# SAIC-MONTREAL/multimodal-dynamics

Measured on AMD Instinct MI355X. Metric: visuotactile samples/sec (train) + ELBO vs CPU ref, cnn-mvae 64x64 bs256 @1/2/4/8 GPU, higher is better.
Workload: dtype f32x3; 1 GPU; cnn-mvae visuotactile+pose 64x64, bs=256 per GPU, fp32 storage and results, GEMMs in the fp32x3 arithmetic (exact three-term bf16 split of the fp32 operands, six of nine products on the bf16 matrix cores, fp32 accumulate; error vs fp64 <= native fp32 MFMA), seq_modeling train step (7 subset ELBOs + backward + Adam), BASELINE configs[1]; global_batch=256, parallelism=dp1, bn=local, launch=hip_graph

## Files before the change

### include/mmdyn_hip.h

```cpp
#ifndef MMDYN_HIP_H
#define MMDYN_HIP_H

#include <stdint.h>

#ifdef __cplusplus
extern "C" {
#endif

#define MMDYN_OK 0
#define MMDYN_ERR_SHAPE (-1)
#define MMDYN_ERR_NULL (-2)
#define MMDYN_ERR_RANGE (-3)

#define MMDYN_ACT_NONE 0
#define MMDYN_ACT_SWISH 1
#define MMDYN_ACT_RELU 2

#define MMDYN_DENSE 0
#define MMDYN_CONV 1
#define MMDYN_TCONV_S2P1 2
#define MMDYN_IM2COL3 3

#define MMDYN_TCONV_S1P0 4

// ... 12 lines not shown
int mmdyn_igemm_nt_dgrad_bn(const float* A, const float* Bp, float* C, float* stats, const float* y,
                            const float* mean, const float* rstd, const float* gamma, const float* beta,
                            int mode, int G, int Bg, int Hi, int Wi, int Cin, int Ho, int Wo, int N,
                            int stride, int offset, int bf16, float* ws, uint32_t* arrival_flags, void* stream);
int mmdyn_igemm_slab_floats(int mode, int G, int Bg, int Hi, int Wi, int Cin, int Ho, int Wo, int N);

int mmdyn_igemm_nt_bf16(const float* A, const float* Bp, const float* bias, float* C, float* C_act,
                        float* stats, float* ws, int mode, int G, int Bg, int Hi, int Wi, int Cin,
                        int Ho, int Wo, int N, int ldc, int stride, int offset, int act, int splitk,
                        void* stream);
int mmdyn_igemm_nt_f16(const float* A, const float* Bp, const float* bias, float* C, float* C_act,
                       float* stats, float* ws, int mode, int G, int Bg, int Hi, int Wi, int Cin,
                       int Ho, int Wo, int N, int ldc, int stride, int offset, int act, int splitk,
                       void* stream);
int mmdyn_igemm_stat_tiles(int mode, int G, int Bg, int Hi, int Wi, int Cin, int Ho, int Wo, int N);
int mmdyn_igemm_stat_tiles_bf16(int mode, int G, int Bg, int Hi, int Wi, int Cin, int Ho, int Wo, int N);
int mmdyn_igemm_stat_tiles_mx(int mode, int G, int Bg, int Hi, int Wi, int Cin, int Ho, int Wo, int N, int flags);
int mmdyn_igemm_slab_floats_mx(int mode, int G, int Bg, int Hi, int Wi, int Cin, int Ho, int Wo, int N, int flags);
int mmdyn_igemm_nt_grouped(const void* A, const void* Bp, const float* bias, void* C, void* C_act, const void* u, int G,
                           int rows, int K, int N, int act, int flags, void* stream);
int mmdyn_splitk_reduce(const float* ws, const float* bias, float* C, float* C_act, int splitk,
                        int rows, int N, int act, void* stream);

int mmdyn_wgrad_tn(const float* D, const float* Gt, float* partial, int mode, int Bt, int Hr, int Wr,
                   int Cd, int Hi, int Wi, int Cg, int stride, int offset, int chunks, void* stream);
int mmdyn_wgrad_tn_bf16(const float* D, const float* Gt, float* partial, int mode, int Bt, int Hr, int Wr,
                        int Cd, int Hi, int Wi, int Cg, int stride, int offset, int chunks, void* stream);
int mmdyn_wgrad_tn_f16(const float* D, const float* Gt, float* partial, int mode, int Bt, int Hr, int Wr,
                       int Cd, int Hi, int Wi, int Cg, int stride, int offset, int chunks, void* stream);
int mmdyn_wgrad_tn_grouped(const void* D, const void* Gt, float* partial, int G, int rows, int Cd, int Cg, int chunks,
                           int flags, void* stream);
int mmdyn_wgrad_out3_bn(const void* y, const float* mean, const float* rstd, const float* gamma, const float* beta,
                        const float* Gt, float* partial, int G, int Bg, int Hr, int chunks, int y_b16, void* stream);
int mmdyn_wgrad_chunks(int mode, int rows, int Cd, int Cg);
int mmdyn_wgrad_chunks_mx(int mode, int rows, int Cd, int Cg, int flags);
int mmdyn_wgrad_reduce(const float* partial, float* canon, int chunks, int taps, int Cd, int Cg,
                       int cg_canon, int perm, float beta, void* stream);

int mmdyn_pack_conv_weight(const float* Wc, float* P, int d0, int d1, int swap, void* stream);
int mmdyn_repack2d(const float* in, float* out, int rows_in, int cols_in, int rows_out, int cols_out,
                   int mode, void* stream);

int mmdyn_repack2d_ld(const float* in, float* out, int rows_in, int cols_in, int rows_out, int cols_out,
                      int ld_out, int mode, void* stream);
int mmdyn_pack_conv_weight_b16(const float* Wc, void* P, int d0, int d1, int swap, int half, void* stream);
int mmdyn_repack2d_ld_b16(const float* in, void* out, int rows_in, int cols_in, int rows_out, int cols_out,
                          int ld_out, int mode, int half, void* stream);
typedef struct {
  const float* src;
  float* dst;
  int kind, rows_in, cols_in, rows_out, cols_out, ld_out;
  int dst_bf16;
} mmdyn_pack_entry;
int mmdyn_pack_plan(const mmdyn_pack_entry* plan_dev, int n, void* stream);

int mmdyn_im2col_nchw3(const float* x, float* col, int Bt, int H, int W, void* stream);
int mmdyn_col2im_k4(const float* col, float* out, int Bt, int Hi, int Wi, int Ho, int Wo, int C,
                    int ldcol, int stride, int pad, int tap_major, void* stream);

int mmdyn_tconv_out3_fwd(const float* a, const float* w, float* out, int Bt, int Hi, int Wi, void* stream);
int mmdyn_tconv_out3_bn_fwd(const void* y, const float* mean, const float* rstd, const float* gamma, const float* beta,
                            const float* w, float* out, int G, int Bg, int Hi, int Wi, int b16, void* stream);
int mmdyn_tconv_out3_bn_bce(const void* y, const float* mean, const float* rstd, const float* gamma, const float* beta,
                            const float* w, float* logits, int logits_group, const float* target, const float* mask,
                            int mask_channels, float* dlogit, double* loss_slots, double* unmasked_slots,
                            const int* slot_of_group, float grad_scale, int G, int Bg, int Hi, int Wi, int b16, void* stream);
// ... 204 lines not shown
```

### multimodal-dynamics_amd/csrc/conv3.hip

```cpp
#include "common.h"

namespace {

struct Conv3Geom {
  int G, Bg, Hi, Wi, Ho, ldc;
  int act, want_act_out, want_stats, w_b16;
  int tiles_per_group;
  const void* bn_y;
  const float* bn_mean;
  const float* bn_rstd;
  const float* bn_gamma;
  const float* bn_beta;
};

#define GLOBAL_AS __attribute__((address_space(1)))
typedef GLOBAL_AS char* gchar_p;
__device__ __forceinline__ gchar_p sgpr_ptr(const void* p) {
  const uint64_t u = reinterpret_cast<uint64_t>(p);
  const uint32_t lo = __builtin_amdgcn_readfirstlane((uint32_t)u), hi = __builtin_amdgcn_readfirstlane((uint32_t)(u >> 32));
  return (gchar_p)(((uint64_t)hi << 32) | lo);
}
template <typename T> __device__ __forceinline__ float gld1(gchar_p p);
template <> __device__ __forceinline__ float gld1<float>(gchar_p p) { return *(GLOBAL_AS const float*)p; }
template <> __device__ __forceinline__ float gld1<bf16_t>(gchar_p p) {
  return __uint_as_float((uint32_t)(*(GLOBAL_AS const bf16_t*)p) << 16);
}
template <> __device__ __forceinline__ float gld1<half_t>(gchar_p p) { return h2f(*(GLOBAL_AS const uint16_t*)p); }
template <typename T> struct store16 { typedef bf16_t type; };
template <> struct store16<half_t> { typedef half_t type; };

constexpr int C3_N = 32;
template <typename T, bool BN, int ACT, int SEGS>
__global__ __launch_bounds__(256) __attribute__((amdgpu_waves_per_eu(4, 4))) void conv3_nt_kernel(
    const float* __restrict__ img, const float* __restrict__ Wp, T* __restrict__ C, T* __restrict__ C_act,
    float* __restrict__ stats, const Conv3Geom g) {
  __shared__ float Ws[32 * 65];
  __shared__ float red[4][2][32];
  const int tid = threadIdx.x, lane = tid & 63;
  const int wave = __builtin_amdgcn_readfirstlane(tid >> 6);
  const int x = lane & 31, h = lane >> 5;
  for (int i = tid; i < 512; i += 256) {
    const f32x4 v = g.w_b16 == 2 ? ld4<half_t>(reinterpret_cast<const half_t*>(Wp) + 4 * i)
                    : g.w_b16 ? ld4<bf16_t>(reinterpret_cast<const bf16_t*>(Wp) + 4 * i)
                              : reinterpret_cast<const f32x4*>(Wp)[i];
    const int n = i >> 4, k = (i & 15) * 4;
    Ws[n * 65 + k + 0] = v[0];
    Ws[n * 65 + k + 1] = v[1];
    Ws[n * 65 + k + 2] = v[2];
    Ws[n * 65 + k + 3] = v[3];
  }
  __syncthreads();
  float bw[24];
  auto load_bw = [&]() {
#pragma unroll
    for (int j = 0; j < 24; ++j) bw[j] = Ws[x * 65 + (j >> 3) * 16 + ((j >> 1) & 3) * 4 + 2 * (j & 1) + h];
  };
  if (!BN) load_bw();

  const float bn_g = BN ? g.bn_gamma[x] : 0.f, bn_b = BN ? g.bn_beta[x] : 0.f;
  const int ntiles = g.G * g.tiles_per_group;

  constexpr int C3_HI = 64 * SEGS, C3_HO = 32 * SEGS;
  constexpr int UNITS = C3_HO * SEGS;
  int xl[2];
#pragma unroll
  for (int q = 0; q < 2; ++q) xl[q] = 2 * x - 1 + 2 * q + h;
  const unsigned voffB = (4 * h * C3_N + x) * sizeof(T);
  constexpr unsigned IMG_B = 3 * C3_HI * C3_HI * sizeof(float);
  constexpr unsigned OROW_B = 32 * C3_N * sizeof(T);

  struct TileAt {
    gchar_p imgb;
    size_t orow;
    int y, seg;
    unsigned xoB[2];
    bool xok[2];
  };
  auto locate = [&](int t) {
    TileAt p;
    const int u = t * 4 + wave;
    const int ib = u / UNITS, rem = u - ib * UNITS;
    p.y = rem / SEGS;
    p.seg = rem - p.y * SEGS;
    p.imgb = sgpr_ptr(reinterpret_cast<const char*>(img) + (size_t)ib * IMG_B + (size_t)p.seg * 256 - 4);
    p.orow = (size_t)u * OROW_B;
#pragma unroll
    for (int q = 0; q < 2; ++q) {
      p.xok[q] = (unsigned)(p.seg * 64 + xl[q]) < (unsigned)C3_HI;
      p.xoB[q] = (unsigned)((p.xok[q] ? xl[q] + 1 : 1) * 4);
    }
    return p;
  };
  auto load_a = [&](const TileAt& p, int j) {
    const int ci = j >> 3, yin = 2 * p.y - 1 + ((j >> 1) & 3);
    const bool yok = (unsigned)yin < (unsigned)C3_HI;
    const gchar_p rowp = p.imgb + (unsigned)((ci * C3_HI + (yok ? yin : 0)) * C3_HI) * 4u;
    return gld1<float>(rowp + p.xoB[j & 1]);
  };
  auto erow = [](int e) { return (unsigned)(((e & 3) + 8 * (e >> 2)) * C3_N * sizeof(T)); };

  float a[24], yv[16];
  int t = blockIdx.x;
  if (t >= ntiles) return;
  TileAt cur = locate(t);
#pragma unroll
  for (int j = 0; j < 24; ++j) a[j] = load_a(cur, j);
  if (BN) {
    const gchar_p yb = sgpr_ptr(reinterpret_cast<const char*>(g.bn_y) + cur.orow) + voffB;
#pragma unroll
    for (int e = 0; e < 16; ++e) yv[e] = gld1<T>(yb + erow(e));
  }
  for (; t < ntiles; t += gridDim.x) {
    const int tn = t + gridDim.x < ntiles ? t + gridDim.x : t;
    const TileAt nxt = locate(tn);
    const int grp = (BN || g.want_stats) ? __builtin_amdgcn_readfirstlane((t / (UNITS / 4)) / g.Bg) : 0;
    if (BN) load_bw();
    float bn_m = 0.f, bn_r = 0.f;
    if (BN) {
      bn_m = g.bn_mean[grp * 32 + x];
      bn_r = g.bn_rstd[grp * 32 + x];
    }
    f32x16 acc;
#pragma unroll
    for (int e = 0; e < 16; ++e) acc[e] = 0.f;
#pragma unroll
    for (int j = 0; j < 24; ++j) {
      const int yin = 2 * cur.y - 1 + ((j >> 1) & 3);
      const bool ok = ((unsigned)yin < (unsigned)C3_HI) & cur.xok[j & 1];
      acc = __builtin_amdgcn_mfma_f32_32x32x2f32(ok ? a[j] : 0.f, bw[j], acc, 0, 0, 0);
      a[j] = load_a(nxt, j);
    }

    const gchar_p cb = sgpr_ptr(reinterpret_cast<const char*>(C) + cur.orow) + voffB;
    const gchar_p ab = sgpr_ptr(reinterpret_cast<const char*>(C_act) + cur.orow) + voffB;
    const gchar_p yb = sgpr_ptr(reinterpret_cast<const char*>(g.bn_y) + nxt.orow) + voffB;
    float cs = 0.f, cq = 0.f;
#pragma unroll
    for (int e = 0; e < 16; ++e) {
      float v = acc[e];
      if (BN) {
        const float xh = (yv[e] - bn_m) * bn_r;
        yv[e] = gld1<T>(yb + erow(e));
        v *= swish_gradf_(bn_g * xh + bn_b);
        cs += v;
        cq += v * xh;
      } else {
        cs += v;
        cq += v * v;
      }
      if (sizeof(T) == 2) {
        const float vn = __shfl_down(v, 1, 64);
        if (!(x & 1)) {
          *(GLOBAL_AS uint32_t*)(cb + erow(e)) = pack2<typename store16<T>::type>(v, vn);
          if (ACT >= 0)
            *(GLOBAL_AS uint32_t*)(ab + erow(e)) = pack2<typename store16<T>::type>(apply_act(v, ACT), apply_act(vn, ACT));
        }
      } else {
        *(GLOBAL_AS float*)(cb + erow(e)) = v;
        if (ACT >= 0) *(GLOBAL_AS float*)(ab + erow(e)) = apply_act(v, ACT);
      }
    }
    if (g.want_stats) {
      cs += __shfl_xor(cs, 32, 64);
      cq += __shfl_xor(cq, 32, 64);
      if (h == 0) {
        red[wave][0][x] = cs;
        red[wave][1][x] = cq;
      }
      __syncthreads();
      if (tid < 32) {
        float s0 = 0.f, q0 = 0.f;
#pragma unroll
        for (int w = 0; w < 4; ++w) {
          s0 += red[w][0][tid];
          q0 += red[w][1][tid];
        }
        const size_t sb = ((size_t)t * 2) * 32 + tid;
        stats[sb] = s0;
        stats[sb + 32] = q0;
      }
      __syncthreads();
    }
    cur = nxt;
  }
}

struct Conv3WgradGeom {
  int Bt, Hr, Hi, Wi;
  int img_rows;
  int rows_per_chunk;
  const float* bn_mean;
  const float* bn_rstd;
  const float* bn_gamma;
  const float* bn_beta;
  int Bg;
// ... 160 lines not shown
  g.bn_gamma = bn_gamma;
  g.bn_beta = bn_beta;
  const int ntiles = G * g.tiles_per_group;
  const dim3 grid(ntiles < CONV3_GRID ? ntiles : CONV3_GRID);
  const int variant = bn_y ? 4 : (C_act ? act : -1);
#define CONV3_LAUNCH(T_, BN_, ACT_, S_)                                                                            \
  hipLaunchKernelGGL((conv3_nt_kernel<T_, BN_, ACT_, S_>), grid, dim3(256), 0, st, A, Bp, (T_*)C, (T_*)C_act, stats, g)
#define CONV3_CASE(V, BN_, ACT_)                                                                                   \
  if (variant == (V)) {                                                                                            \
    if (c_b16 == 2) {                                                                                              \
      if (segs == 1) CONV3_LAUNCH(half_t, BN_, ACT_, 1);                                                           \
      else if (segs == 2) CONV3_LAUNCH(half_t, BN_, ACT_, 2);                                                      \
      else CONV3_LAUNCH(half_t, BN_, ACT_, 4);                                                                     \
    } else if (c_b16) {                                                                                            \
      if (segs == 1) CONV3_LAUNCH(bf16_t, BN_, ACT_, 1);                                                           \
      else if (segs == 2) CONV3_LAUNCH(bf16_t, BN_, ACT_, 2);                                                      \
      else CONV3_LAUNCH(bf16_t, BN_, ACT_, 4);                                                                     \
    } else {                                                                                                       \
      if (segs == 1) CONV3_LAUNCH(float, BN_, ACT_, 1);                                                            \
      else if (segs == 2) CONV3_LAUNCH(float, BN_, ACT_, 2);                                                       \
      else CONV3_LAUNCH(float, BN_, ACT_, 4);                                                                      \
    }                                                                                                              \
  }
  CONV3_CASE(4, true, -1)
  CONV3_CASE(-1, false, -1)
  CONV3_CASE(MMDYN_ACT_NONE, false, MMDYN_ACT_NONE)
  CONV3_CASE(MMDYN_ACT_SWISH, false, MMDYN_ACT_SWISH)
  CONV3_CASE(MMDYN_ACT_RELU, false, MMDYN_ACT_RELU)
#undef CONV3_LAUNCH
#undef CONV3_CASE
  MMDYN_LAUNCH_CHECK();
}

int mmdyn_conv3_wgrad_try(const void* D, const float* Gt, float* partial, int Bt, int Hr, int Wr, int Cd, int Hi,
                          int Wi, int Cg, int chunks, int d_b16, hipStream_t st, const float* bn_mean, const float* bn_rstd,
                          const float* bn_gamma, const float* bn_beta, int Bg) {
  if (Cd != 32 || Cg != 64 || Wr != Hr || Wi != Hi || Hi != 2 * Hr || (Hi != 64 && Hi != 128 && Hi != 256)) return 1;
  const int segs = Hi / 64;
  if ((int64_t)Bt * Hr * segs >= (1LL << 30)) return 1;
  Conv3WgradGeom g{};
  g.Bt = Bt;
  g.Hr = Hr;
  g.Hi = Hi;
  g.Wi = Wi;
  g.img_rows = Bt * Hr * segs;
  g.rows_per_chunk = ceil_div(g.img_rows, chunks);
  g.bn_mean = bn_mean;
  g.bn_rstd = bn_rstd;
  g.bn_gamma = bn_gamma;
  g.bn_beta = bn_beta;
  g.Bg = Bg > 0 ? Bg : Bt;
#define CONV3_WG(T_, S_)                                                                                                  \
  do {                                                                                                                    \
    if (bn_mean)                                                                                                          \
      hipLaunchKernelGGL((conv3_wgrad_kernel<T_, S_, true>), dim3(chunks), dim3(256), 0, st, (const T_*)D, Gt, partial, g); \
    else                                                                                                                  \
      hipLaunchKernelGGL((conv3_wgrad_kernel<T_, S_>), dim3(chunks), dim3(256), 0, st, (const T_*)D, Gt, partial, g);     \
  } while (0)
  if (d_b16 == 2) {
    if (segs == 1) CONV3_WG(half_t, 1);
    else if (segs == 2) CONV3_WG(half_t, 2);
    else CONV3_WG(half_t, 4);
  } else if (d_b16) {
    if (segs == 1) CONV3_WG(bf16_t, 1);
    else if (segs == 2) CONV3_WG(bf16_t, 2);
    else CONV3_WG(bf16_t, 4);
// ... 9 lines not shown
```

### multimodal-dynamics_amd/mmdyn_hip/_lib.py

```python
import ctypes
import os

_HERE = os.path.dirname(os.path.abspath(__file__))
LIB_PATH = os.environ.get("MMDYN_HIP_LIB") or os.path.join(_HERE, "libmmdyn_hip.so")

_P, _I, _L, _F, _Q = ctypes.c_void_p, ctypes.c_int, ctypes.c_int64, ctypes.c_float, ctypes.c_uint64


class PassExperts(ctypes.Structure):
    _fields_ = [("mu", _P * 4), ("lv", _P * 4), ("dmu", _P * 4), ("dlv", _P * 4), ("ld", _I * 4), ("dz", _P * 3),
                ("zdst", _P * 3), ("zpl", _P * 3)]


class PackEntry(ctypes.Structure):
    _fields_ = [("src", _P), ("dst", _P), ("kind", _I), ("rows_in", _I), ("cols_in", _I), ("rows_out", _I),
                ("cols_out", _I), ("ld_out", _I), ("dst_bf16", _I)]


class FeedGroups(ctypes.Structure):
    _fields_ = [("recon", _P * 4), ("obs", _P * 4), ("out", _P * 4), ("row_len", _I * 4), ("logits", _I * 4), ("column", _I * 4)]


MAX_PASSES = 8
MAX_EXPERTS = 4
# ... 3 lines not shown
_SIGNATURES = {
    "mmdyn_abi_version": "",
    "mmdyn_igemm_nt": "ppppppp" + "iiiiiiiiiiiiii" + "p",
    "mmdyn_igemm_nt_dgrad_bn": "ppppppppp" + "iiiiiiiiiiii" + "ppp",
    "mmdyn_igemm_nt_dgrad_act": "pppp" + "i" + "iiiiiiiiiii" + "i" + "ppp",
    "mmdyn_igemm_slab_floats": "iiiiiiiii",
    "mmdyn_igemm_nt_bf16": "ppppppp" + "iiiiiiiiiiiiii" + "p",
    "mmdyn_igemm_nt_f16": "ppppppp" + "iiiiiiiiiiiiii" + "p",
    "mmdyn_igemm_stat_tiles": "iiiiiiiii",
    "mmdyn_igemm_stat_tiles_bf16": "iiiiiiiii",
    "mmdyn_igemm_stat_tiles_mx": "iiiiiiiiii",
    "mmdyn_igemm_slab_floats_mx": "iiiiiiiiii",
    "mmdyn_igemm_nt_grouped": "pppppp" + "iiiiii" + "p",
    "mmdyn_splitk_reduce": "pppp" + "iiii" + "p",
    "mmdyn_wgrad_tn": "ppp" + "iiiiiiiiiii" + "p",
    "mmdyn_wgrad_tn_bf16": "ppp" + "iiiiiiiiiii" + "p",
    "mmdyn_wgrad_tn_f16": "ppp" + "iiiiiiiiiii" + "p",
    "mmdyn_wgrad_tn_grouped": "ppp" + "iiiiii" + "p",
    "mmdyn_wgrad_chunks": "iiii",
    "mmdyn_wgrad_chunks_mx": "iiiii",
    "mmdyn_wgrad_reduce": "pp" + "iiiiii" + "f" + "p",
    "mmdyn_pack_conv_weight": "pp" + "iii" + "p",
    "mmdyn_repack2d": "pp" + "iiiii" + "p",
    "mmdyn_repack2d_ld": "pp" + "iiiiii" + "p",
    "mmdyn_pack_conv_weight_b16": "pp" + "iiii" + "p",
    "mmdyn_repack2d_ld_b16": "pp" + "iiiiiii" + "p",
    "mmdyn_pack_plan": "p" + "i" + "p",
    "mmdyn_im2col_nchw3": "pp" + "iii" + "p",
    "mmdyn_col2im_k4": "pp" + "iiiiiiiiii" + "p",
    "mmdyn_tconv_out3_fwd": "ppp" + "iii" + "p",
    "mmdyn_tconv_out3_bn_fwd": "ppppppp" + "iiiii" + "p",
    "mmdyn_tconv_out3_bn_bce": "ppppppp" + "i" + "pp" + "i" + "pppp" + "f" + "iiiii" + "p",
    "mmdyn_wgrad_out3_bn": "ppppppp" + "iiiii" + "p",
    "mmdyn_colstats": "pp" + "iii" + "p",
    "mmdyn_colstats_tiles": "i",
    "mmdyn_bn_finalize": "ppppppp" + "iiii" + "ff" + "i" + "pp",
    "mmdyn_bn_swish_fwd": "pppppp" + "iii" + "p",
    "mmdyn_bn_swish_bwd_reduce": "ppppppp" + "iii" + "p",
    "mmdyn_bn_bwd_finalize": "ppppp" + "iii" + "f" + "pp",
    "mmdyn_bn_eval_stats": "pppp" + "ii" + "f" + "p",
    "mmdyn_bn_reduce_partials": "ppp" + "iii" + "p",
    "mmdyn_bn_finalize_sums": "pppppp" + "iii" + "ff" + "i" + "p",
    "mmdyn_bn_bwd_finalize_sums": "pppp" + "ii" + "ff" + "p",
    "mmdyn_bn_swish_bwd_apply": "pppppppp" + "iiii" + "p",
    "mmdyn_act_fwd": "pp" + "l" + "i" + "p",
    "mmdyn_act_bwd": "ppp" + "l" + "i" + "p",
    "mmdyn_dropout_expand": "ppp" + "iii" + "f" + "p",
    "mmdyn_dropout_reduce": "ppp" + "iii" + "f" + "pi" + "pp",
    "mmdyn_random_masks": "p" + "l" + "f" + "QQ" + "pp",
    "mmdyn_random_normal": "p" + "l" + "QQ" + "pp",
    "mmdyn_counter_add": "p" + "Q" + "p",
    "mmdyn_colsum": "ppp" + "iii" + "f" + "pp",
    "mmdyn_colsum_chunks": "i",
    "mmdyn_scale_dev": "ppp" + "l" + "p",
    "mmdyn_sum_blocks": "pp" + "i" + "l" + "p",
    "mmdyn_copy_many": "ppp" + "i" + "p",
    "mmdyn_cast_f32_to_bf16": "pp" + "l" + "p",
    "mmdyn_cast_bf16_to_f32": "pp" + "l" + "p",
    "mmdyn_linear_small_fwd": "pppp" + "iiii" + "p",
    "mmdyn_linear_small_bwd": "pppppp" + "iii" + "f" + "p",
    "mmdyn_poe_fwd": "pppppp" + "iiii" + "p",
    "mmdyn_poe_bwd": "ppppppp" + "f" + "iiii" + "pp",
    "mmdyn_reparam_fwd": "ppppp" + "iii" + "p",
    "mmdyn_reparam_bwd": "pppp" + "f" + "pp" + "iii" + "p",
    "mmdyn_bce_logits": "ppppp" + "l" + "iii" + "f" + "p",
    "mmdyn_bce_logits_groups": "ppppp" + "i" + "l" + "f" + "p",
# ... 89 lines not shown
```

### multimodal-dynamics_amd/mmdyn_hip/layers.py

```python
import weakref

import torch

from . import ops
from .ops import ACT_NONE, ACT_SWISH, ACT_RELU, DENSE, CONV, TCONV_S2P1, IM2COL3, TCONV_S1P0
from .models.shapes import BN_EPS, BN_MOMENTUM, FEAT


def _new(like, *shape, dtype=torch.float32):
    if isinstance(like, ops.Planes):
        like = like.t
    return torch.empty(shape, device=like.device, dtype=dtype)


ACT_DTYPE = torch.float32
W_DTYPE = torch.float32


def _act(like, *shape):
    return torch.empty(shape, device=like.device, dtype=ACT_DTYPE)


def _cdiv(a, b):
    return (a + b - 1) // b
# ... 233 lines not shown


def _eval_mode_check():
    if SYNC is not None:
        raise RuntimeError("mmdyn_hip: the eval-mode backward normalises with the local running estimates; it does not run under "
                           "a synchronised BatchNorm (layers.SYNC must be None)")


def _bn_eval_param_grads(y, partial, T, dgamma, dbeta, G, C):
    ops.B.bn_bwd_finalize(partial, _new(y, G, 2, C), dgamma, dbeta, _new(y, 32, G, 2, C, dtype=torch.float64), G, T, C, 0.0)


def bn_swish_backward(da, y, mean, rstd, bn, dgamma, dbeta, G, rows_per_group, C, planes_out=False, eval_mode=False):
    T = ops.B.colstats_tiles(rows_per_group)
    if eval_mode:
        _eval_mode_check()
        partial = _new(y, G, T, 2, C) if (dgamma is not None or dbeta is not None) else None
        dy, dyp = _apply_out(y, planes_out)
        ops.backend_op("bn_eval_swish_bwd")(da, y, mean, rstd, bn.gamma, bn.beta, dy, partial, G, rows_per_group, C, False, planes=dyp)
        if partial is not None:
            _bn_eval_param_grads(y, partial, T, dgamma, dbeta, G, C)
        return dy if dyp is None else dyp
    partial = _new(y, G, T, 2, C)
    ops.B.bn_swish_bwd_reduce(da, y, mean, rstd, bn.gamma, bn.beta, partial, G, rows_per_group, C)
    sums = _bn_backward_sums(y, partial, T, dgamma, dbeta, G, C)
    dy, dyp = _apply_out(y, planes_out)
    if dyp is not None:
        ops.B.bn_swish_bwd_apply(da, y, mean, rstd, bn.gamma, bn.beta, sums, None, G, rows_per_group, C, planes=dyp)
        return dyp
    ops.B.bn_swish_bwd_apply(da, y, mean, rstd, bn.gamma, bn.beta, sums, dy, G, rows_per_group, C)
    return dy


def dgrad_bn_swish_backward(x, Wp, mode, G, Bg, Hi, Cin, Ho, N, stride, offset, y, mean, rstd, bn, dgamma, dbeta, planes_out=False,
                            eval_mode=False):
    rows_per_group = Bg * Ho * Ho
    if eval_mode:
        _eval_mode_check()
    if y.dtype == torch.float32 and mode != IM2COL3:
        x, Wp = split_operands(x, Wp, mode, G, Bg, Hi, Cin, Ho, N)
    if isinstance(x, ops.Planes):
        T = ops.B.igemm_stat_tiles(mode, G, Bg, Hi, Hi, Cin, Ho, Ho, N, planes=True)
    else:
        T = ops.B.igemm_stat_tiles(mode, G, Bg, Hi, Hi, Cin, Ho, Ho, N, all16=ops._is16(x) and ops._is16(Wp))
    du = torch.empty_like(y)
    partial = _new(y, G, T, 2, N)
    ops.B.igemm_nt_dgrad_bn(x, Wp, du, partial, y, mean, rstd, bn.gamma, bn.beta, mode, G, Bg, Hi, Hi, Cin, Ho, Ho, N,
                            stride, offset)
    if eval_mode:
        if dgamma is not None or dbeta is not None:
            _bn_eval_param_grads(y, partial, T, dgamma, dbeta, G, N)
        dy, dyp = _apply_out(y, planes_out)
        ops.backend_op("bn_eval_swish_bwd")(du, None, mean, rstd, bn.gamma, bn.beta, dy, None, G, rows_per_group, N, True, planes=dyp)
        return dy if dyp is None else dyp
    sums = _bn_backward_sums(y, partial, T, dgamma, dbeta, G, N)
    dy, dyp = _apply_out(y, planes_out)
    if dyp is not None:
        ops.B.bn_swish_bwd_apply(du, y, mean, rstd, bn.gamma, bn.beta, sums, None, G, rows_per_group, N, True, planes=dyp)
        return dyp
    ops.B.bn_swish_bwd_apply(du, y, mean, rstd, bn.gamma, bn.beta, sums, dy, G, rows_per_group, N, True)
    return dy


def wgrad(D, Gt, canon, mode, Bt, Hr, Cd, Hi, Cg, stride=1, offset=0, cg_canon=None, perm=0, defer=None):
    if defer is not None:
        defer.append((D, Gt, canon, mode, Bt, Hr, Cd, Hi, Cg, stride, offset, cg_canon, perm))
        return
    rows = Bt * Hr * Hr
    taps = 16 if mode == CONV else 1
    if isinstance(D, ops.Planes) or isinstance(Gt, ops.Planes):
        chunks = ops.B.wgrad_chunks(mode, rows, Cd, Cg, planes=(isinstance(D, ops.Planes), isinstance(Gt, ops.Planes)))
    else:
        chunks = ops.B.wgrad_chunks(mode, rows, Cd, Cg)
    partial = _new(D, chunks, taps, Cd, Cg)
    ops.B.wgrad_tn(D, Gt, partial, mode, Bt, Hr, Hr, Cd, Hi, Hi, Cg, stride, offset, chunks)
    ops.B.wgrad_reduce(partial, canon, chunks, taps, Cd, Cg, Cg if cg_canon is None else cg_canon, perm, 0.0)

# ... 690 lines not shown
```

### multimodal-dynamics_amd/mmdyn_hip/ops.py

```python
import ctypes

import os

import torch

from . import _lib
from ._lib import PassExperts, FeedGroups, MAX_PASSES, MAX_EXPERTS, FEED_GROUPS, check

ACT_NONE, ACT_SWISH, ACT_RELU = 0, 1, 2
DENSE, CONV, TCONV_S2P1, IM2COL3, TCONV_S1P0 = 0, 1, 2, 3, 4
ROW_GROUPS_MAX = 8


def _ptr(t, dtype=torch.float32):
    if t is None:
        return None
    if not t.is_cuda:
        raise RuntimeError("mmdyn_hip: the HIP path needs GPU tensors (got a CPU tensor); there is no CPU fallback")
    if t.dtype != dtype:
        raise TypeError(f"mmdyn_hip: expected {dtype}, got {t.dtype}")
    if not t.is_contiguous():
        raise ValueError("mmdyn_hip: tensor must be contiguous")
    return t.data_ptr()

# ... 428 lines not shown
            raise ValueError("mmdyn_hip: tconv_out3_bn_bce: dlogit buffer of the wrong size")
        if mask is not None and tuple(mask.shape) != (Bg, mask_channels, 2 * Hi, 2 * Wi):
            raise ValueError(f"mmdyn_hip: tconv_out3_bn_bce: mask {tuple(mask.shape)} is not [Bg][{mask_channels}][2Hi][2Wi]")
        slots = (ctypes.c_int * G)(*[int(s) for s in slot_of_group])
        check(self.lib.mmdyn_tconv_out3_bn_bce(py, _ptr(mean), _ptr(rstd), _ptr(gamma), _ptr(beta), _ptr(w), _ptr(logits),
                                               int(logits_group), _ptr(target), _ptr(mask), int(mask_channels), _ptr(dlogit),
                                               loss_slots.data_ptr(), None if unmasked_slots is None else unmasked_slots.data_ptr(),
                                               ctypes.addressof(slots), float(grad_scale), G, Bg, Hi, Wi, y16, _stream()),
              "mmdyn_tconv_out3_bn_bce")

    def tconv_out3_bn_bce_rows(self, y, mean, rstd, gamma, beta, w, logits, logits_group, target, loss_rows, slot_of_group, G, Bg,
                               Hi, Wi, mask=None, mask_channels=1, unmasked_rows=None):
        py, y16 = _aptr(y)
        if len(slot_of_group) != G or tuple(target.shape) != (Bg, 3, 2 * Hi, 2 * Wi):
            raise ValueError("mmdyn_hip: tconv_out3_bn_bce_rows: one slot per group and a [Bg][3][2Hi][2Wi] target")
        if logits is not None and logits.numel() != (G if logits_group < 0 else 1) * Bg * 3 * 4 * Hi * Wi:
            raise ValueError("mmdyn_hip: tconv_out3_bn_bce_rows: logits buffer of the wrong size")
        if mask is not None and tuple(mask.shape) != (Bg, mask_channels, 2 * Hi, 2 * Wi):
            raise ValueError(f"mmdyn_hip: tconv_out3_bn_bce_rows: mask {tuple(mask.shape)} is not [Bg][{mask_channels}][2Hi][2Wi]")
        n_slots = self._row_slots(loss_rows, Bg, "tconv_out3_bn_bce_rows")
        if unmasked_rows is not None and self._row_slots(unmasked_rows, Bg, "tconv_out3_bn_bce_rows") != n_slots:
            raise ValueError("mmdyn_hip: tconv_out3_bn_bce_rows: unmasked_rows and loss_rows differ in shape")
        slots = (ctypes.c_int * G)(*[int(s) for s in slot_of_group])
        check(self.lib.mmdyn_tconv_out3_bn_bce_rows(py, _ptr(mean), _ptr(rstd), _ptr(gamma), _ptr(beta), _ptr(w), _ptr(logits),
                                                    int(logits_group), _ptr(target), _ptr(mask), int(mask_channels),
                                                    _ptr(loss_rows, torch.float64), _ptr(unmasked_rows, torch.float64),
                                                    ctypes.addressof(slots), n_slots, G, Bg, Hi, Wi, y16, _stream()),
              "mmdyn_tconv_out3_bn_bce_rows")

    def wgrad_out3_bn(self, y, mean, rstd, gamma, beta, Gt, partial, G, Bg, Hr, chunks):
        py, y16 = _aptr(y)
        check(self.lib.mmdyn_wgrad_out3_bn(py, _ptr(mean), _ptr(rstd), _ptr(gamma), _ptr(beta), _ptr(Gt), _ptr(partial), G, Bg, Hr,
                                           chunks, y16, _stream()), "mmdyn_wgrad_out3_bn")

    def nchw_to_nhwc(self, src, dst, B, C, HW):
        check(self.lib.mmdyn_nchw_to_nhwc(_ptr(src), _ptr(dst), B, C, HW, _stream()), "mmdyn_nchw_to_nhwc")

    def nhwc_to_nchw(self, src, dst, B, C, HW):
        check(self.lib.mmdyn_nhwc_to_nchw(_ptr(src), _ptr(dst), B, C, HW, _stream()), "mmdyn_nhwc_to_nchw")

    def colstats(self, y, partial, G, rows_per_group, C):
        check(self.lib.mmdyn_colstats(_ptr(y), _ptr(partial), G, rows_per_group, C, _stream()), "mmdyn_colstats")

    def bn_finalize(self, partial, mean, rstd, running_mean, running_var, nbt, scratch, G, T, C, rows_per_group,
                    eps, momentum, repeat):
        check(self.lib.mmdyn_bn_finalize(_ptr(partial), _ptr(mean), _ptr(rstd), _ptr(running_mean),
                                         _ptr(running_var), _ptr(nbt, torch.int64), _ptr(scratch, torch.float64),
                                         G, T, C, rows_per_group, eps, momentum, repeat, self._ticket(partial, G * T), _stream()),
              "mmdyn_bn_finalize")

    def bn_swish_fwd(self, y, mean, rstd, gamma, beta, a, G, rows_per_group, C, planes=None):
        if planes is not None:
            if planes.rows != G * rows_per_group or planes.C != C:
                raise ValueError("mmdyn_hip: bn_swish_fwd: plane tensor of the wrong shape")
            check(self.lib.mmdyn_bn_swish_fwd_planes(_ptr(y), _ptr(mean), _ptr(rstd), _ptr(gamma), _ptr(beta), _ptr(a),
                                                     planes.t.data_ptr(), G, rows_per_group, C, _stream()), "mmdyn_bn_swish_fwd_planes")
            return
        (py, y16), (pa, a16) = _aptr(y), _aptr(a)
        if y16 != a16:
            raise TypeError("mmdyn_hip: bn_swish_fwd input and output must share the storage type")
        if y16:
            check(self.lib.mmdyn_bn_swish_fwd_b16(py, _ptr(mean), _ptr(rstd), _ptr(gamma), _ptr(beta), pa, G, rows_per_group, C,
                                                  _half(y16), _stream()), "mmdyn_bn_swish_fwd_b16")
            return
        check(self.lib.mmdyn_bn_swish_fwd(py, _ptr(mean), _ptr(rstd), _ptr(gamma), _ptr(beta), pa, G, rows_per_group, C,
                                          _stream()), "mmdyn_bn_swish_fwd")
# ... 543 lines not shown
```

### multimodal-dynamics_amd/mmdyn_hip/profiling.py

```python
import collections

import torch

from . import ops

PAD_CYCLES = 100000
HOST_ONLY = {"igemm_stat_tiles", "colstats_tiles", "wgrad_chunks", "igemm_planes_served"}


def _canon(name, a):
    if name == "igemm_nt_dgrad_bn":
        A, Bp, C, stats, y, mean, rstd, gamma, beta, mode, G, Bg, Hi, Wi, Cin, Ho, Wo, N, stride, offset = a
        name, a = "igemm_nt", (A, Bp, y, C, None, stats, None, mode, G, Bg, Hi, Wi, Cin, Ho, Wo, N, N, stride, offset, 0, 1)
    if name == "igemm_nt_dgrad_act":
        A, Bp, C, u, act, mode, G, Bg, Hi, Wi, Cin, Ho, Wo, N, stride, offset = a
        name, a = "igemm_nt", (A, Bp, u, C, None, None, None, mode, G, Bg, Hi, Wi, Cin, Ho, Wo, N, N, stride, offset, 0, 1)
    if name == "igemm_nt_grouped":
        A, Bp, bias, C, C_act, u, G, rows, K, N, act = a
        name, a = "igemm_nt", (A, Bp, bias if u is None else u, C, C_act, None, None, ops.DENSE, G, rows, 1, 1, K, 1, 1, N, N, 1, 0, act, 1)
    if name == "wgrad_tn_grouped":
        D, Gt, partial, G, rows, Cd, Cg, chunks = a
        name, a = "wgrad_tn", (D, Gt, partial, ops.DENSE, G * rows, 1, 1, Cd, 1, 1, Cg, 1, 0, chunks)
    if name == "wgrad_out3_bn":
        y, mean, rstd, gamma, beta, Gt, partial, G, Bg, Hr, chunks = a
        return "conv3_wgrad", (y, Gt, partial, ops.IM2COL3, G * Bg, Hr, Hr, 32, 2 * Hr, 2 * Hr, 64, 1, 0, chunks)
    if name == "tconv_out3_bn_fwd":
        return "tconv_out3_fwd", a
    if name == "igemm_nt" and a[7] == ops.IM2COL3 and a[10] in (64, 128, 256) and \
            tuple(a[10:17]) == (a[10], a[10], 64, a[10] // 2, a[10] // 2, 32, 32):
        return "conv3_nt", a
    if name == "igemm_nt" and a[7] == ops.TCONV_S2P1 and tuple(a[10:16]) in ((16, 16, 64, 32, 32, 32), (32, 32, 32, 64, 64, 32),
                                                                            (64, 64, 32, 128, 128, 32)) and \
            getattr(ops.B, "precision", "fp32") == "fp32" and all(not torch.is_tensor(t) or t.dtype == torch.float32 for t in a[:4]):
        return "tconv_patch", a
    if name == "wgrad_tn" and a[3] == ops.IM2COL3 and a[8] in (64, 128, 256) and \
            tuple(a[5:11]) == (a[8] // 2, a[8] // 2, 32, a[8], a[8], 64):
        return "conv3_wgrad", a
    return name, a


def _flops(name, a):
    if name in ("igemm_nt", "conv3_nt", "tconv_patch"):
        (mode, G, Bg, Hi, Wi, Cin, Ho, Wo, N) = a[7:16]
        if mode == ops.DENSE:
            return 2.0 * G * Bg * Ho * Wo * N * Cin
        if mode == ops.CONV:
            return 2.0 * G * Bg * Ho * Wo * N * 16 * Cin
        if mode == ops.TCONV_S1P0:
            return 2.0 * G * Bg * Hi * Wi * N * 16 * Cin
        if mode == ops.IM2COL3:
            return 2.0 * G * Bg * Ho * Wo * N * 48
        return 2.0 * G * Bg * Ho * Wo * N * 4 * Cin
    if name in ("wgrad_tn", "conv3_wgrad"):
        (mode, Bt, Hr, Wr, Cd, Hi, Wi, Cg) = a[3:11]
        return 2.0 * Bt * Hr * Wr * Cd * Cg * (16 if mode == ops.CONV else 1)
    return 0.0


def _bytes(a):
    n = 0
    for t in a:
        if isinstance(t, ops.Planes):
            t = t.t
        if torch.is_tensor(t):
            n += t.numel() * t.element_size()
    return n


class TimedBackend:
    name = "hip"

    def __init__(self, inner):
        self._inner = inner
        self.records = []

    @property
    def precision(self):
        return self._inner.precision

    @precision.setter
    def precision(self, value):
        self._inner.precision = value

    @property
    def fp32_split(self):
        return getattr(self._inner, "fp32_split", False)

    @fp32_split.setter
    def fp32_split(self, value):
        self._inner.fp32_split = value

    def __getattr__(self, attr):
        fn = getattr(self._inner, attr)
        if attr in HOST_ONLY or not callable(fn):
            return fn

        def wrapped(*a, **k):
            s, e = torch.cuda.Event(enable_timing=True), torch.cuda.Event(enable_timing=True)
            torch.cuda._sleep(PAD_CYCLES)
            s.record()
            r = fn(*a, **k)
            e.record()
            name, ca = _canon(attr, a)
            sig = tuple(x for x in ca if isinstance(x, (int, bool))) if name in ("igemm_nt", "wgrad_tn", "conv3_nt", "conv3_wgrad", "tconv_patch") else ()
            if attr == "igemm_nt_dgrad_bn":
                sig = sig + ("bn_bwd_epilogue",)
            if attr == "igemm_nt_dgrad_act":
                sig = sig + ("act_bwd_epilogue",)
            if attr in ("igemm_nt_grouped", "wgrad_tn_grouped"):
                sig = sig + ("grouped",)
            self.records.append((name, _flops(name, ca), _bytes(ca), s, e, sig))
            return r
        return wrapped

    def summary(self):
        torch.cuda.synchronize()
        agg = collections.OrderedDict()
        self.by_shape = collections.OrderedDict()
        for name, fl, by, s, e, sig in self.records:
            if sig:
                d2 = self.by_shape.setdefault((name,) + sig, {"calls": 0, "ms": 0.0, "flops": 0.0})
                d2["calls"] += 1
                d2["ms"] += s.elapsed_time(e)
                d2["flops"] += fl
            d = agg.setdefault(name, {"calls": 0, "ms": 0.0, "flops": 0.0, "bytes": 0.0})
            d["calls"] += 1
            d["ms"] += s.elapsed_time(e)
            d["flops"] += fl
            d["bytes"] += by
        return agg


def profile_step(fn):
    timed = TimedBackend(ops.B)
    old = ops.set_backend(timed)
    try:
# ... 7 lines not shown
```

Baseline: 52030 samples/s.

## Recompute out3 dgrad in two passes to fuse BN-backward apply

```diff
diff --git a/include/mmdyn_hip.h b/include/mmdyn_hip.h
--- a/include/mmdyn_hip.h
+++ b/include/mmdyn_hip.h
@@ -68,6 +68,11 @@
                            int flags, void* stream);
 int mmdyn_wgrad_out3_bn(const void* y, const float* mean, const float* rstd, const float* gamma, const float* beta,
                         const float* Gt, float* partial, int G, int Bg, int Hr, int chunks, int y_b16, void* stream);
+int mmdyn_out3_bwd_stats(const float* dlogits, const float* Wp, float* stats, const float* y, const float* mean, const float* rstd,
+                         const float* gamma, const float* beta, int G, int Bg, int Hi, void* stream);
+int mmdyn_out3_bwd_apply(const float* dlogits, const float* Wp, const float* y, const float* mean, const float* rstd,
+                         const float* gamma, const float* beta, const float* sums, float* dy, void* dy_planes, int G, int Bg,
+                         int Hi, void* stream);
 int mmdyn_wgrad_chunks(int mode, int rows, int Cd, int Cg);
 int mmdyn_wgrad_chunks_mx(int mode, int rows, int Cd, int Cg, int flags);
 int mmdyn_wgrad_reduce(const float* partial, float* canon, int chunks, int taps, int Cd, int Cg,
diff --git a/multimodal-dynamics_amd/csrc/conv3.hip b/multimodal-dynamics_amd/csrc/conv3.hip
--- a/multimodal-dynamics_amd/csrc/conv3.hip
+++ b/multimodal-dynamics_amd/csrc/conv3.hip
@@ -11,6 +11,8 @@
   const float* bn_rstd;
   const float* bn_gamma;
   const float* bn_beta;
+  const float* bn_sums;
+  float inv_n;
 };
 
 #define GLOBAL_AS __attribute__((address_space(1)))
@@ -30,12 +32,18 @@
 template <> struct store16<half_t> { typedef half_t type; };
 
 constexpr int C3_N = 32;
-template <typename T, bool BN, int ACT, int SEGS>
+constexpr int C3_OUT_C = 0, C3_OUT_NONE = 1, C3_OUT_DY = 2, C3_OUT_PLANES = 3, C3_OUT_PLANES_PAIRED = 4;
+constexpr int C3_TP_LD = 36;
+template <typename T, bool BN, int ACT, int SEGS, int OUT = C3_OUT_C>
 __global__ __launch_bounds__(256) __attribute__((amdgpu_waves_per_eu(4, 4))) void conv3_nt_kernel(
     const float* __restrict__ img, const float* __restrict__ Wp, T* __restrict__ C, T* __restrict__ C_act,
     float* __restrict__ stats, const Conv3Geom g) {
   __shared__ float Ws[32 * 65];
   __shared__ float red[4][2][32];
+  static_assert(OUT == C3_OUT_C || (BN && sizeof(T) == 4 && ACT < 0), "the two-pass forms are fp32 BatchNorm-backward variants");
+  constexpr bool APPLY = OUT >= C3_OUT_DY;
+  constexpr bool VIA_LDS = OUT == C3_OUT_DY || OUT == C3_OUT_PLANES;
+  __shared__ __attribute__((aligned(16))) float tpatch[VIA_LDS ? 4 * 32 * C3_TP_LD : 4];
   const int tid = threadIdx.x, lane = tid & 63;
   const int wave = __builtin_amdgcn_readfirstlane(tid >> 6);
   const int x = lane & 31, h = lane >> 5;
@@ -68,6 +76,7 @@
   const unsigned voffB = (4 * h * C3_N + x) * sizeof(T);
   constexpr unsigned IMG_B = 3 * C3_HI * C3_HI * sizeof(float);
   constexpr unsigned OROW_B = 32 * C3_N * sizeof(T);
+  constexpr unsigned PROW_B = 3 * C3_N * sizeof(bf16_t);
 
   struct TileAt {
     gchar_p imgb;
@@ -134,6 +143,12 @@
     const gchar_p cb = sgpr_ptr(reinterpret_cast<const char*>(C) + cur.orow) + voffB;
     const gchar_p ab = sgpr_ptr(reinterpret_cast<const char*>(C_act) + cur.orow) + voffB;
     const gchar_p yb = sgpr_ptr(reinterpret_cast<const char*>(g.bn_y) + nxt.orow) + voffB;
+    float ap_s0 = 0.f, ap_s1 = 0.f, ap_gr = 0.f;
+    if constexpr (APPLY) {
+      ap_s0 = g.bn_sums[(grp * 2 + 0) * 32 + x] * g.inv_n;
+      ap_s1 = g.bn_sums[(grp * 2 + 1) * 32 + x] * g.inv_n;
+      ap_gr = bn_g * bn_r;
+    }
     float cs = 0.f, cq = 0.f;
 #pragma unroll
     for (int e = 0; e < 16; ++e) {
@@ -141,14 +156,37 @@
       if (BN) {
         const float xh = (yv[e] - bn_m) * bn_r;
         yv[e] = gld1<T>(yb + erow(e));
-        v *= swish_gradf_(bn_g * xh + bn_b);
-        cs += v;
-        cq += v * xh;
+        if constexpr (OUT == C3_OUT_C) {
+          v *= swish_gradf_(bn_g * xh + bn_b);
+          cs += v;
+          cq += v * xh;
+        } else {
+          v *= swish_gradf_(bn_g * xh + bn_b);
+          asm("" : "+v"(v));
+          cs += v;
+          cq += v * xh;
+        }
+        if constexpr (APPLY) v = ap_gr * (v - ap_s0 - xh * ap_s1);
       } else {
         cs += v;
         cq += v * v;
       }
-      if (sizeof(T) == 2) {
+      if constexpr (OUT == C3_OUT_NONE) {
+      } else if constexpr (VIA_LDS) {
+        tpatch[(wave * 32 + (e & 3) + 8 * (e >> 2) + 4 * h) * C3_TP_LD + x] = v;
+      } else if constexpr (OUT == C3_OUT_PLANES_PAIRED) {
+        const float vn = __shfl_down(v, 1, 64);
+        if (!(x & 1)) {
+          const gchar_p pb = sgpr_ptr(reinterpret_cast<const char*>(C) + (size_t)(t * 4 + wave) * (32 * PROW_B)) +
+                             (unsigned)(4 * h * PROW_B + x * sizeof(bf16_t));
+          const unsigned po = ((e & 3) + 8 * (e >> 2)) * PROW_B;
+          uint32_t ph, pm, pl;
+          split3_bf16(v, vn, ph, pm, pl);
+          *(GLOBAL_AS uint32_t*)(pb + po) = ph;
+          *(GLOBAL_AS uint32_t*)(pb + po + C3_N * sizeof(bf16_t)) = pm;
+          *(GLOBAL_AS uint32_t*)(pb + po + 2 * C3_N * sizeof(bf16_t)) = pl;
+        }
+      } else if (sizeof(T) == 2) {
         const float vn = __shfl_down(v, 1, 64);
         if (!(x & 1)) {
           *(GLOBAL_AS uint32_t*)(cb + erow(e)) = pack2<typename store16<T>::type>(v, vn);
@@ -160,7 +198,32 @@
         if (ACT >= 0) *(GLOBAL_AS float*)(ab + erow(e)) = apply_act(v, ACT);
       }
     }
-    if (g.want_stats) {
+    if constexpr (VIA_LDS) {
+      __builtin_amdgcn_wave_barrier();
+      const gchar_p fb = sgpr_ptr(reinterpret_cast<const char*>(C) + cur.orow) + (unsigned)(lane * 8 * sizeof(float));
+      const gchar_p pb = sgpr_ptr(reinterpret_cast<const char*>(C) + (size_t)(t * 4 + wave) * (32 * PROW_B)) +
+                         (unsigned)((lane >> 2) * PROW_B + (lane & 3) * 8 * sizeof(bf16_t));
+#pragma unroll
+      for (int i = 0; i < 2; ++i) {
+        const float* src = tpatch + (wave * 32 + (lane >> 2) + 16 * i) * C3_TP_LD + (lane & 3) * 8;
+        const f32x4 va = *reinterpret_cast<const f32x4*>(src), vb = *reinterpret_cast<const f32x4*>(src + 4);
+        if constexpr (OUT == C3_OUT_DY) {
+          *(GLOBAL_AS f32x4*)(fb + i * 16 * C3_N * sizeof(float)) = va;
+          *(GLOBAL_AS f32x4*)(fb + i * 16 * C3_N * sizeof(float) + 16) = vb;
+          continue;
+        }
+        uint32_t h0, h1, h2, h3, m0, m1, m2, m3, l0, l1, l2, l3;
+        split3_bf16(va[0], va[1], h0, m0, l0);
+        split3_bf16(va[2], va[3], h1, m1, l1);
+        split3_bf16(vb[0], vb[1], h2, m2, l2);
+        split3_bf16(vb[2], vb[3], h3, m3, l3);
+        *(GLOBAL_AS u32x4_t*)(pb + 16 * i * PROW_B) = u32x4_t{h0, h1, h2, h3};
+        *(GLOBAL_AS u32x4_t*)(pb + 16 * i * PROW_B + C3_N * sizeof(bf16_t)) = u32x4_t{m0, m1, m2, m3};
+        *(GLOBAL_AS u32x4_t*)(pb + 16 * i * PROW_B + 2 * C3_N * sizeof(bf16_t)) = u32x4_t{l0, l1, l2, l3};
+      }
+      __builtin_amdgcn_wave_barrier();
+    }
+    if (!APPLY && g.want_stats) {
       cs += __shfl_xor(cs, 32, 64);
       cq += __shfl_xor(cq, 32, 64);
       if (h == 0) {
@@ -387,6 +450,71 @@
   MMDYN_LAUNCH_CHECK();
 }
 
+static int out3_bwd_launch(int out, const float* dlogits, const float* Wp, void* dst, float* stats, const float* y,
+                           const float* mean, const float* rstd, const float* gamma, const float* beta, const float* sums, int G,
+                           int Bg, int Hi, hipStream_t st) {
+  if (!dlogits || !Wp || !y || !mean || !rstd || !gamma || !beta) return MMDYN_ERR_NULL;
+  if (out == C3_OUT_NONE ? !stats : (!dst || !sums)) return MMDYN_ERR_NULL;
+  if (G < 1 || Bg < 1 || (Hi != 64 && Hi != 128 && Hi != 256)) return MMDYN_ERR_SHAPE;
+  const int Ho = Hi / 2, segs = Hi / 64;
+  if ((int64_t)G * Bg * Hi * Hi * 3 >= (1LL << 31) || (int64_t)G * Bg * Ho * Ho * C3_N >= (1LL << 31)) return MMDYN_ERR_RANGE;
+  Conv3Geom g{};
+  g.G = G;
+  g.Bg = Bg;
+  g.Hi = Hi;
+  g.Wi = Hi;
+  g.Ho = Ho;
+  g.ldc = C3_N;
+  g.act = MMDYN_ACT_NONE;
+  g.want_stats = out == C3_OUT_NONE;
+  g.tiles_per_group = Bg * Ho * Ho / 128;
+  g.bn_y = y;
+  g.bn_mean = mean;
+  g.bn_rstd = rstd;
+  g.bn_gamma = gamma;
+  g.bn_beta = beta;
+  g.bn_sums = sums;
+  g.inv_n = 1.f / (float)(Bg * Ho * Ho);
+  const int ntiles = G * g.tiles_per_group;
+  const dim3 grid(ntiles < CONV3_GRID ? ntiles : CONV3_GRID);
+#ifdef MMDYN_LAB
+  if (out == C3_OUT_PLANES && lab_env("MMDYN_OUT3_PAIRED")) out = C3_OUT_PLANES_PAIRED;
+#endif
+#define OUT3_LAUNCH(S_, O_)                                                                                              \
+  hipLaunchKernelGGL((conv3_nt_kernel<float, true, -1, S_, O_>), grid, dim3(256), 0, st, dlogits, Wp, (float*)dst,     \
+                     (float*)nullptr, stats, g)
+#define OUT3_CASE(O_)                                                                                                    \
+  if (out == (O_)) {                                                                                                     \
+    if (segs == 1) OUT3_LAUNCH(1, O_);                                                                                   \
+    else if (segs == 2) OUT3_LAUNCH(2, O_);                                                                              \
+    else OUT3_LAUNCH(4, O_);                                                                                             \
+  }
+  OUT3_CASE(C3_OUT_NONE)
+  OUT3_CASE(C3_OUT_DY)
+  OUT3_CASE(C3_OUT_PLANES)
+#ifdef MMDYN_LAB
+  OUT3_CASE(C3_OUT_PLANES_PAIRED)
+#endif
+#undef OUT3_LAUNCH
+#undef OUT3_CASE
+  MMDYN_LAUNCH_CHECK();
+}
+
+extern "C" int mmdyn_out3_bwd_stats(const float* dlogits, const float* Wp, float* stats, const float* y, const float* mean,
+                                    const float* rstd, const float* gamma, const float* beta, int G, int Bg, int Hi,
+                                    void* stream) {
+  return out3_bwd_launch(C3_OUT_NONE, dlogits, Wp, nullptr, stats, y, mean, rstd, gamma, beta, nullptr, G, Bg, Hi,
+                         (hipStream_t)stream);
+}
+
+extern "C" int mmdyn_out3_bwd_apply(const float* dlogits, const float* Wp, const float* y, const float* mean, const float* rstd,
+                                    const float* gamma, const float* beta, const float* sums, float* dy, void* dy_planes, int G,
+                                    int Bg, int Hi, void* stream) {
+  if ((dy != nullptr) == (dy_planes != nullptr)) return dy ? MMDYN_ERR_SHAPE : MMDYN_ERR_NULL;
+  return out3_bwd_launch(dy ? C3_OUT_DY : C3_OUT_PLANES, dlogits, Wp, dy ? (void*)dy : dy_planes, nullptr, y, mean, rstd, gamma,
+                         beta, sums, G, Bg, Hi, (hipStream_t)stream);
+}
+
 int mmdyn_conv3_wgrad_try(const void* D, const float* Gt, float* partial, int Bt, int Hr, int Wr, int Cd, int Hi,
                           int Wi, int Cg, int chunks, int d_b16, hipStream_t st, const float* bn_mean, const float* bn_rstd,
                           const float* bn_gamma, const float* bn_beta, int Bg) {
diff --git a/multimodal-dynamics_amd/mmdyn_hip/_lib.py b/multimodal-dynamics_amd/mmdyn_hip/_lib.py
--- a/multimodal-dynamics_amd/mmdyn_hip/_lib.py
+++ b/multimodal-dynamics_amd/mmdyn_hip/_lib.py
@@ -59,6 +59,8 @@
     "mmdyn_tconv_out3_bn_fwd": "ppppppp" + "iiiii" + "p",
     "mmdyn_tconv_out3_bn_bce": "ppppppp" + "i" + "pp" + "i" + "pppp" + "f" + "iiiii" + "p",
     "mmdyn_wgrad_out3_bn": "ppppppp" + "iiiii" + "p",
+    "mmdyn_out3_bwd_stats": "pppppppp" + "iii" + "p",
+    "mmdyn_out3_bwd_apply": "pppppppppp" + "iii" + "p",
     "mmdyn_colstats": "pp" + "iii" + "p",
     "mmdyn_colstats_tiles": "i",
     "mmdyn_bn_finalize": "ppppppp" + "iiii" + "ff" + "i" + "pp",
diff --git a/multimodal-dynamics_amd/mmdyn_hip/layers.py b/multimodal-dynamics_amd/mmdyn_hip/layers.py
--- a/multimodal-dynamics_amd/mmdyn_hip/layers.py
+++ b/multimodal-dynamics_amd/mmdyn_hip/layers.py
@@ -289,6 +289,11 @@
     return dy
 
 
+def out3_two_pass(x, Wp, mode, y, eval_mode):
+    return (mode == IM2COL3 and not eval_mode and y.dtype == torch.float32 and torch.is_tensor(x) and x.dtype == torch.float32
+            and Wp.dtype == torch.float32 and getattr(ops.B, "out3_bwd_stats", None) is not None)
+
+
 def dgrad_bn_swish_backward(x, Wp, mode, G, Bg, Hi, Cin, Ho, N, stride, offset, y, mean, rstd, bn, dgamma, dbeta, planes_out=False,
                             eval_mode=False):
     rows_per_group = Bg * Ho * Ho
@@ -300,6 +305,13 @@
         T = ops.B.igemm_stat_tiles(mode, G, Bg, Hi, Hi, Cin, Ho, Ho, N, planes=True)
     else:
         T = ops.B.igemm_stat_tiles(mode, G, Bg, Hi, Hi, Cin, Ho, Ho, N, all16=ops._is16(x) and ops._is16(Wp))
+    if out3_two_pass(x, Wp, mode, y, eval_mode):
+        partial = _new(y, G, T, 2, N)
+        ops.B.out3_bwd_stats(x, Wp, partial, y, mean, rstd, bn.gamma, bn.beta, G, Bg, Hi)
+        sums = _bn_backward_sums(y, partial, T, dgamma, dbeta, G, N)
+        dy, dyp = _apply_out(y, planes_out)
+        ops.B.out3_bwd_apply(x, Wp, y, mean, rstd, bn.gamma, bn.beta, sums, dy, G, Bg, Hi, planes=dyp)
+        return dy if dyp is None else dyp
     du = torch.empty_like(y)
     partial = _new(y, G, T, 2, N)
     ops.B.igemm_nt_dgrad_bn(x, Wp, du, partial, y, mean, rstd, bn.gamma, bn.beta, mode, G, Bg, Hi, Hi, Cin, Ho, Ho, N,
diff --git a/multimodal-dynamics_amd/mmdyn_hip/ops.py b/multimodal-dynamics_amd/mmdyn_hip/ops.py
--- a/multimodal-dynamics_amd/mmdyn_hip/ops.py
+++ b/multimodal-dynamics_amd/mmdyn_hip/ops.py
@@ -484,6 +484,33 @@
         py, y16 = _aptr(y)
         check(self.lib.mmdyn_wgrad_out3_bn(py, _ptr(mean), _ptr(rstd), _ptr(gamma), _ptr(beta), _ptr(Gt), _ptr(partial), G, Bg, Hr,
                                            chunks, y16, _stream()), "mmdyn_wgrad_out3_bn")
+
+    @staticmethod
+    def _out3_bwd_shapes(name, dlogits, Wp, y, mean, rstd, gamma, beta, G, Bg, Hi):
+        rows = G * Bg * (Hi // 2) ** 2
+        want = ((dlogits, G * Bg * 3 * Hi * Hi), (Wp, 32 * 64), (y, rows * 32), (mean, G * 32), (rstd, G * 32), (gamma, 32), (beta, 32))
+        if Hi not in (64, 128, 256) or any(t.numel() != n for t, n in want):
+            raise ValueError(f"mmdyn_hip: {name}: tensor sizes do not belong to G = {G}, Bg = {Bg}, Hi = {Hi}")
+        return rows
+
+    def out3_bwd_stats(self, dlogits, Wp, stats, y, mean, rstd, gamma, beta, G, Bg, Hi):
+        rows = self._out3_bwd_shapes("out3_bwd_stats", dlogits, Wp, y, mean, rstd, gamma, beta, G, Bg, Hi)
+        if tuple(stats.shape) != (G, rows // G // 128, 2, 32):
+            raise ValueError(f"mmdyn_hip: out3_bwd_stats: stats must be [G={G}][T={rows // G // 128}][2][32], got {tuple(stats.shape)}")
+        check(self.lib.mmdyn_out3_bwd_stats(_ptr(dlogits), _ptr(Wp), _ptr(stats), _ptr(y), _ptr(mean), _ptr(rstd), _ptr(gamma),
+                                            _ptr(beta), G, Bg, Hi, _stream()), "mmdyn_out3_bwd_stats")
+
+    def out3_bwd_apply(self, dlogits, Wp, y, mean, rstd, gamma, beta, sums, dy, G, Bg, Hi, planes=None):
+        rows = self._out3_bwd_shapes("out3_bwd_apply", dlogits, Wp, y, mean, rstd, gamma, beta, G, Bg, Hi)
+        if sums.numel() != G * 2 * 32 or (dy is None) == (planes is None):
+            raise ValueError("mmdyn_hip: out3_bwd_apply: sums must be [G][2][32], and exactly one of dy / planes is written")
+        if planes is not None and (planes.rows != rows or planes.C != 32 or not planes.t.is_cuda or not planes.t.is_contiguous()):
+            raise ValueError("mmdyn_hip: out3_bwd_apply: plane tensor of the wrong shape")
+        if dy is not None and dy.numel() != rows * 32:
+            raise ValueError("mmdyn_hip: out3_bwd_apply: dy of the wrong shape")
+        check(self.lib.mmdyn_out3_bwd_apply(_ptr(dlogits), _ptr(Wp), _ptr(y), _ptr(mean), _ptr(rstd), _ptr(gamma), _ptr(beta),
+                                            _ptr(sums), _ptr(dy), None if planes is None else planes.t.data_ptr(), G, Bg, Hi,
+                                            _stream()), "mmdyn_out3_bwd_apply")
 
     def nchw_to_nhwc(self, src, dst, B, C, HW):
         check(self.lib.mmdyn_nchw_to_nhwc(_ptr(src), _ptr(dst), B, C, HW, _stream()), "mmdyn_nchw_to_nhwc")
diff --git a/multimodal-dynamics_amd/mmdyn_hip/profiling.py b/multimodal-dynamics_amd/mmdyn_hip/profiling.py
--- a/multimodal-dynamics_amd/mmdyn_hip/profiling.py
+++ b/multimodal-dynamics_amd/mmdyn_hip/profiling.py
@@ -51,6 +51,9 @@
         if mode == ops.IM2COL3:
             return 2.0 * G * Bg * Ho * Wo * N * 48
         return 2.0 * G * Bg * Ho * Wo * N * 4 * Cin
+    if name in ("out3_bwd_stats", "out3_bwd_apply"):
+        G, Bg, Hi = a[8:11] if name == "out3_bwd_stats" else a[9:12]
+        return 2.0 * G * Bg * (Hi // 2) ** 2 * 32 * 48
     if name in ("wgrad_tn", "conv3_wgrad"):
         (mode, Bt, Hr, Wr, Cd, Hi, Wi, Cg) = a[3:11]
         return 2.0 * Bt * Hr * Wr * Cd * Cg * (16 if mode == ops.CONV else 1)
@@ -102,6 +105,8 @@
             r = fn(*a, **k)
             e.record()
             name, ca = _canon(attr, a)
+            if attr == "out3_bwd_apply" and k.get("planes") is not None:
+                ca = ca + (k["planes"],)
             sig = tuple(x for x in ca if isinstance(x, (int, bool))) if name in ("igemm_nt", "wgrad_tn", "conv3_nt", "conv3_wgrad", "tconv_patch") else ()
             if attr == "igemm_nt_dgrad_bn":
                 sig = sig + ("bn_bwd_epilogue",)
```

New measurement: 52340 samples/s, median of 6. About the same (+0.6%).
